# XiangFeng-Wen/STF-Unet

Measured on AMD Instinct MI355X. Metric: training samples/sec (256x256 DCE-MRI frames), higher is better.
Workload: dtype bf16; 1 GPU; cfg2 UNet(in=8,base_c=64) 256x256 train step; model=UNet, global_batch=64, per_gpu_batch=64, seq_len=8, parallelism=dp1, ddp_hook=False

## Files before the change

### include/stfunet.h

```cpp
#ifndef STFUNET_H
#define STFUNET_H
#include <stddef.h>
#include <stdint.h>

#ifdef __cplusplus
extern "C" {
#endif

typedef void* stf_stream_t;

typedef struct stf_conv_geom {
  int N;
  int Hs, Ws, Cs;
  int src_cstride;
  int Hd, Wd;
  int R, S;
  int stride, pad;
  int transposed;
} stf_conv_geom;

typedef struct stf_lstm_epi {
  const float* c_prev;
  float* c_out;
  void* h_out;
// ... 347 lines not shown
  int cx, cy, kx, ky;
  int oh, ow, h0, w0;
  int flags;
  int fx[6];
  int pad_;
  double m[6];
} stf_aug_frame;
int stf_augment_frames(const uint8_t* src, const stf_aug_frame* frames, int n, const int* coef,
                       uint8_t* scratch, int max_resized_px, int max_out_px, float mean, float stdv,
                       float* out, stf_stream_t stream);
int stf_augment_masks(const uint8_t* src, const stf_aug_frame* masks, int n, const int* tabs,
                      int max_out_px, int64_t* out, stf_stream_t stream);

typedef struct stf_plan stf_plan;
stf_plan* stf_plan_create(void);
void stf_plan_destroy(stf_plan* plan);
int stf_plan_record(stf_plan* plan);
int stf_plan_stop(void);
int stf_plan_size(const stf_plan* plan);
int stf_plan_tag(const char* name, double flops);
int stf_plan_tag_end(void);
int stf_plan_replay(stf_plan* plan, int first, int last, const char* timed_tag);
int stf_plan_timing(stf_plan* plan, int* launches, double* ms, double* flops);
int stf_stream_wait(stf_stream_t waiter, stf_stream_t waitee);
int stf_memset(void* p, int value, size_t bytes, stf_stream_t stream);
int stf_copy_rows(const float* src, int64_t src_ld, float* dst, int64_t dst_ld, int rows, int cols,
                  stf_stream_t stream);
int stf_i64_add_batch(int64_t* const* ptrs, int count, int64_t inc, stf_stream_t stream);

const char* stf_error_string(int code);
int stf_abi_version(void);

#define STF_STORAGE_BF16 0
#define STF_STORAGE_FP16 1
int stf_storage_type(void);

#ifdef __cplusplus
}
#endif
#endif
```

### stf-unet_amd/csrc/common.h

```cpp
#pragma once
#include <hip/hip_runtime.h>
#include <stdint.h>

#include <tuple>
#include <type_traits>
#include <utility>

#ifdef STF_FP16
typedef _Float16 e16;
#else
typedef __bf16 e16;
#endif
typedef e16 e16x8 __attribute__((ext_vector_type(8)));
typedef e16 e16x4 __attribute__((ext_vector_type(4)));
typedef short short4v __attribute__((ext_vector_type(4)));
typedef float f32x4 __attribute__((ext_vector_type(4)));
typedef float f32x16 __attribute__((ext_vector_type(16)));
typedef unsigned int u32x4v __attribute__((ext_vector_type(4)));

#define STF_DEV __device__ __forceinline__

STF_DEV float e2f(e16 v) { return (float)v; }
STF_DEV e16 f2e(float v) { return (e16)v; }

// ... 103 lines not shown
  return v;
}

template <typename T>
STF_DEV T wave_max(T v) {
#pragma unroll
  for (int o = 32; o > 0; o >>= 1) {
    const T t = __shfl_xor(v, o, 64);
    v = t > v ? t : v;
  }
  return v;
}
template <typename T>
STF_DEV T wave_min(T v) {
#pragma unroll
  for (int o = 32; o > 0; o >>= 1) {
    const T t = __shfl_xor(v, o, 64);
    v = t < v ? t : v;
  }
  return v;
}

namespace stf {
struct PlanOp {
  virtual ~PlanOp() {}
  virtual hipError_t run() const = 0;
};
bool plan_recording();
void plan_append(PlanOp* op, hipStream_t s);

template <class... A>
struct KernelOp final : PlanOp {
  const void* fn;
  dim3 grid, block;
  unsigned shmem;
  hipStream_t stream;
  std::tuple<A...> args;
  template <class... B>
  KernelOp(const void* f, dim3 g, dim3 b, unsigned sh, hipStream_t s, B&&... a)
      : fn(f), grid(g), block(b), shmem(sh), stream(s), args(std::forward<B>(a)...) {}
  hipError_t run() const override {
    return std::apply(
        [this](const A&... a) {
          void* p[sizeof...(A) + 1] = {const_cast<void*>(static_cast<const void*>(&a))...};
          return hipLaunchKernel(fn, grid, block, p, shmem, stream);
        },
        args);
  }
};

template <class... A, class... B>
inline void launch(void (*k)(A...), dim3 g, dim3 b, unsigned sh, hipStream_t s, B&&... args) {
  static_assert(sizeof...(A) == sizeof...(B), "kernel argument count");
  if (!plan_recording()) {
    std::tuple<std::decay_t<A>...> t(std::forward<B>(args)...);
    std::apply(
        [&](auto&... a) {
          void* p[sizeof...(A) + 1] = {static_cast<void*>(&a)...};
          (void)hipLaunchKernel((const void*)k, g, b, p, sh, s);
        },
        t);
    return;
  }
  auto* op = new KernelOp<std::decay_t<A>...>((const void*)k, g, b, sh, s, std::forward<B>(args)...);
  (void)op->run();
  plan_append(op, s);
}

hipError_t memset_async(void* p, int value, size_t bytes, hipStream_t s);
char ab_letter(const char* name);
hipError_t memcpy_async(void* dst, const void* src, size_t bytes, hipMemcpyKind kind, hipStream_t s);
// ... 25 lines not shown
```

### stf-unet_amd/csrc/head.hip

```cpp
#include "common.h"
#include "../../include/stfunet.h"
#include "reduce.h"

namespace {

constexpr int NT = 256;

STF_DEV float lane_group_sum(float v, int CG) {
  if (CG >= 2) v += dpp_f<0xB1>(v);
  if (CG >= 4) v += dpp_f<0x4E>(v);
  if (CG >= 8) v += dpp_f<0x141>(v);
  if (CG >= 16) v += dpp_f<0x140>(v);
  for (int o = 16; o < CG; o <<= 1) v += __shfl_xor(v, o, 64);
  return v;
}

int head_tiles(long units) {
  long t = (units + NT - 1) / NT;
  return (int)(t < 1 ? 1 : (t > 1024 ? 1024 : t));
}

template <int K>
__global__ void head_fwd_kernel(const uint16_t* __restrict__ y, long P, int HW, int C,
                                const float* __restrict__ scale, const float* __restrict__ shift,
// ... 345 lines not shown

extern "C" int stf_head_fwd(const void* y, int N, int H, int W, int C, const float* scale, const float* shift,
                            const float* w, const float* bias, int classes, float* logits, stf_stream_t stream) {
  if (!head_ok(C)) return STF_EINVAL;
  const long P = (long)N * H * W, units = P * (C / 8);
  if (units >= (1L << 31)) return STF_EINVAL;
  long blocks = (units + NT - 1) / NT;
  if (blocks > 8192) blocks = 8192;
  hipStream_t s = (hipStream_t)stream;
  STF_KDISPATCH(classes, hipLaunchKernelGGL(head_fwd_kernel<KK>, dim3(blocks), dim3(NT), 0, s, (const uint16_t*)y,
                                            P, H * W, C, scale, shift, w, bias, logits));
  STF_CHECK_LAUNCH();
  return 0;
}

extern "C" int stf_head_bwd(const float* dlogits, const void* y, int N, int H, int W, int C, const float* scale,
                            const float* shift, const float* mean, const float* invstd, const float* w, int classes,
                            void* g_out, float* bn_partial, float* head_partial, float* dw, float* db,
                            stf_stream_t stream) {
  if (!head_ok(C) || (long)N * H * W * (C / 8) >= (1L << 31)) return STF_EINVAL;
  const long P = (long)N * H * W;
  const int tiles = stf_head_tiles(N, H, W, C);
  hipStream_t s = (hipStream_t)stream;
  STF_KDISPATCH(classes, hipLaunchKernelGGL(head_bwd_kernel<KK>, dim3(tiles), dim3(NT), 0, s, dlogits,
                                            (const uint16_t*)y, P, H * W, C, scale, shift, mean, invstd, w,
                                            (uint16_t*)g_out, bn_partial, head_partial));
  STF_CHECK_LAUNCH();
  const int HC = classes * (C + 1);
  const int S = stf::colsum_stage1(head_partial, tiles, HC, s);
  hipLaunchKernelGGL(sum_tiles_kernel, dim3((HC + 255) / 256), dim3(256), 0, s, head_partial, S, HC, classes * C,
                     dw, db);
  STF_CHECK_LAUNCH();
  return 0;
}

extern "C" int stf_head_mc_fwd(const void* y, int N, int H, int W, int C, const float* scale, const float* shift,
                               const float* w, const float* bias, int classes, float* logits, stf_stream_t stream) {
  if (C < 8 || !head_ok(C) || !mc_classes_ok(classes) || N < 1 || H < 1 || W < 1) return STF_EINVAL;
  if (!y || !scale || !shift || !w || !bias || !logits) return STF_EINVAL;
  const long P = (long)N * H * W, units = P * (C / 8);
  if (!head_mc_units_ok((long)H * W, units)) return STF_EINVAL;
  long blocks = (units + NT - 1) / NT;
  if (blocks > MCBLOCKS) blocks = MCBLOCKS;
  hipStream_t s = (hipStream_t)stream;
  STF_KPDISPATCH(classes, hipLaunchKernelGGL(head_mc_fwd_kernel<KP>, dim3(blocks), dim3(NT),
                                             head_mc_lds_bytes(C, classes, false), s, (const uint16_t*)y, P, H * W, C,
// ... 30 lines not shown
```

### stf-unet_amd/csrc/loss.hip

```cpp
#include "common.h"
#include "../../include/stfunet.h"
#include <cmath>

namespace {

constexpr int NT = 256;
constexpr int MAXK = 4;
constexpr int MCK = 16;
constexpr int LCHUNK = 64;
constexpr float DICE_EPS = 1e-6f;

template <bool OPT> struct LossOpt { static constexpr int dice = 1; };
template <> struct LossOpt<true> { const float* cw; int ignore, dice; };

template <int K, bool OPT, class... O>
__global__ void loss_fwd_kernel(const float* __restrict__ logits, const int64_t* __restrict__ target, int HW,
                                float* __restrict__ part, O... opt) {
  constexpr int NV = 3 * K + 1 + OPT;
  const LossOpt<OPT> o{opt...};
  __shared__ float red[NT / 64][NV];
  const int n = blockIdx.y;
  float w[K];
  if constexpr (OPT) {
#pragma unroll
// ... 25 lines not shown
      s[3 * k] += p * tk;
      s[3 * k + 1] += p;
      s[3 * k + 2] += tk;
      if (t == k) {
        const float nll = lse - (z[k] - mx);
        if constexpr (OPT) { s[3 * K] += w[k] * nll; s[3 * K + 1] += w[k]; }
        else s[3 * K] += nll;
      }
    }
  }
#pragma unroll
  for (int i = 0; i < NV; ++i) s[i] = wave_sum(s[i]);
  if ((threadIdx.x & 63) == 0)
#pragma unroll
    for (int i = 0; i < NV; ++i) red[threadIdx.x >> 6][i] = s[i];
  __syncthreads();
  if (threadIdx.x < NV) {
    float a = 0.f;
    for (int wv = 0; wv < NT / 64; ++wv) a += red[wv][threadIdx.x];
    part[((size_t)n * gridDim.x + blockIdx.x) * NV + threadIdx.x] = a;
  }
}

template <int K, bool OPT>
__global__ void loss_finalize_kernel(const float* __restrict__ part, int N, int hw_or_dice, float* __restrict__ terms,
                                     float* __restrict__ loss) {
  constexpr int NV = 3 * K + 1 + OPT;
  __shared__ double acc[64][NV];
  double ce = 0.0, wsum = 0.0, dsum = 0.0;
  for (int base = 0; base < N; base += 64) {
    const int n = base + (int)threadIdx.x;
    if (threadIdx.x < 64) {
      for (int i = 0; i < NV; ++i) {
        double a = 0.0;
        if (n < N)
          for (int c = 0; c < LCHUNK; ++c) a += part[((size_t)n * LCHUNK + c) * NV + i];
        acc[threadIdx.x][i] = a;
      }
    }
    __syncthreads();
    if (threadIdx.x == 0) {
      for (int r = 0; r < 64 && base + r < N; ++r) {
        for (int k = 0; k < K; ++k) {
          const double I = acc[r][3 * k], S = acc[r][3 * k + 1] + acc[r][3 * k + 2];
          const float If = (float)I, Sf = (float)S;
          const float setsum = Sf == 0.f ? 2.f * If : Sf;
          dsum += (double)((2.f * If + DICE_EPS) / (setsum + DICE_EPS));
          terms[((size_t)(base + r) * K + k) * 3 + 0] = If;
          terms[((size_t)(base + r) * K + k) * 3 + 1] = (float)acc[r][3 * k + 1];
          terms[((size_t)(base + r) * K + k) * 3 + 2] = (float)acc[r][3 * k + 2];
        }
        ce += acc[r][3 * K];
        if constexpr (OPT) wsum += acc[r][3 * K + 1];
      }
    }
    __syncthreads();
  }
  if (threadIdx.x == 0) {
    terms[(size_t)N * K * 3] = (float)ce;
    if constexpr (OPT) {
      terms[(size_t)N * K * 3 + 1] = (float)wsum;
      loss[0] = (float)(ce / wsum + (hw_or_dice ? 1.0 - dsum / ((double)N * K) : 0.0));
    } else {
      loss[0] = (float)(ce / ((double)N * hw_or_dice) + 1.0 - dsum / ((double)N * K));
    }
  }
}

template <int K, bool OPT, class... O>
__global__ void loss_bwd_kernel(const float* __restrict__ logits, const int64_t* __restrict__ target, int N, int HW,
                                const float* __restrict__ terms, const float* __restrict__ grad_out,
                                float* __restrict__ dlogits, O... opt) {
  const LossOpt<OPT> o{opt...};
  const long P = (long)N * HW;
  const float go = grad_out ? grad_out[0] : 1.f;
  float inv_den = 1.f / (float)P;
// ... 109 lines not shown
    }
  }
  s[3 * KP] = wave_sum(s[3 * KP]);
  s[3 * KP + 1] = wave_sum(s[3 * KP + 1]);
#pragma unroll
  for (int i = 0; i < 3 * KP; ++i)
    if (i < 3 * K) s[i] = wave_sum(s[i]);
  if ((threadIdx.x & 63) == 0) {
#pragma unroll
    for (int i = 0; i < 3 * KP; ++i)
      if (i < 3 * K) red[threadIdx.x >> 6][i] = s[i];
    red[threadIdx.x >> 6][3 * K] = s[3 * KP];
    red[threadIdx.x >> 6][3 * K + 1] = s[3 * KP + 1];
  }
  __syncthreads();
  if ((int)threadIdx.x < NV) {
    float a = 0.f;
    for (int wv = 0; wv < NT / 64; ++wv) a += red[wv][threadIdx.x];
    part[((size_t)n * gridDim.x + blockIdx.x) * NV + threadIdx.x] = a;
  }
}

template <bool FT, class... F>
__global__ __launch_bounds__(NT) void loss_mc_finalize_kernel(const float* __restrict__ part, int N, int K, int dice,
                                                              F... ft, float* __restrict__ terms,
                                                              float* __restrict__ loss) {
  constexpr int NVM = 3 * MCK + 2;
  __shared__ double acc[64][NVM];
  __shared__ double dk[64][MCK], drow[64];
  const int NV = 3 * K + 2, r = threadIdx.x & 63, q = threadIdx.x >> 6;
  double ce = 0.0, wsum = 0.0, dsum = 0.0;
  for (int base = 0; base < N; base += 64) {
    const int n = base + r, rows = N - base < 64 ? N - base : 64;
    for (int i = q; i < NV; i += NT / 64) {
      double a = 0.0;
      if (n < N)
        for (int c = 0; c < LCHUNK; ++c) a += part[((size_t)n * LCHUNK + c) * NV + i];
      acc[r][i] = a;
    }
    __syncthreads();
    for (int e = threadIdx.x; e < rows * K; e += NT) {
      const int rr = e / K, k = e - rr * K;
      if constexpr (FT) {
        const LossFT o{0.f, ft...};
        const float I = (float)acc[rr][3 * k], P = (float)acc[rr][3 * k + 1], T = (float)acc[rr][3 * k + 2];
        const float den = 2.f * (1.f - o.alpha - o.beta) * I + 2.f * o.alpha * P + 2.f * o.beta * T + DICE_EPS;
        dk[rr][k] = (P + T == 0.f) ? 1.0 : (double)((2.f * I + DICE_EPS) / den);
        float* tp = terms + ((size_t)(base + rr) * K + k) * 3;
        tp[0] = I;
        tp[1] = P;
        tp[2] = T;
      } else {
        const double I = acc[rr][3 * k], S = acc[rr][3 * k + 1] + acc[rr][3 * k + 2];
        const float If = (float)I, Sf = (float)S;
        const float setsum = Sf == 0.f ? 2.f * If : Sf;
        dk[rr][k] = (double)((2.f * If + DICE_EPS) / (setsum + DICE_EPS));
        float* tp = terms + ((size_t)(base + rr) * K + k) * 3;
        tp[0] = If;
        tp[1] = (float)acc[rr][3 * k + 1];
        tp[2] = (float)acc[rr][3 * k + 2];
      }
    }
    __syncthreads();
    if ((int)threadIdx.x < rows) {
// ... 102 lines not shown
    }
#pragma unroll
    for (int k = 0; k < KP; ++k) {
      if (k < K) {
        const float tk = t == k ? 1.f : 0.f;
        const float G = (t == k ? ga[k] : 0.f) + gb[k];
        const float g = go * ((z[k] - tk) * cs + z[k] * (G - pg));
        dp[(size_t)k * HW + hw] = keep ? g : 0.f;
      }
    }
  }
}

int loss_scratch_floats(int N, int K, bool opt) { return N * K * 3 + 1 + opt + N * LCHUNK * (3 * K + 1 + opt); }

template <bool OPT, class... O>
int loss_fwd(const float* logits, const int64_t* target, int N, int HW, int classes, float* terms, float* loss,
             hipStream_t s, O... opt) {
  float* part = terms + N * classes * 3 + 1 + OPT;
  const int hw_or_dice = OPT ? LossOpt<OPT>{opt...}.dice : HW;
  STF_KDISPATCH(classes, {
    hipLaunchKernelGGL((loss_fwd_kernel<KK, OPT, O...>), dim3(LCHUNK, N), dim3(NT), 0, s, logits, target, HW, part,
                       opt...);
    hipLaunchKernelGGL((loss_finalize_kernel<KK, OPT>), dim3(1), dim3(64), 0, s, part, N, hw_or_dice, terms, loss);
  });
  STF_CHECK_LAUNCH();
  return 0;
}

template <bool OPT, class... O>
int loss_bwd(const float* logits, const int64_t* target, int N, int HW, int classes, const float* terms,
             const float* grad_out, float* dlogits, hipStream_t s, O... opt) {
  const long P = (long)N * HW;
  long blocks = (P + NT - 1) / NT;
  if (blocks > 8192) blocks = 8192;
  STF_KDISPATCH(classes, hipLaunchKernelGGL((loss_bwd_kernel<KK, OPT, O...>), dim3(blocks), dim3(NT), 0, s, logits,
                                            target, N, HW, terms, grad_out, dlogits, opt...));
  STF_CHECK_LAUNCH();
  return 0;
}

bool loss_opt_ok(int classes, int ignore_index) {
  return classes >= 1 && classes <= MAXK && !(ignore_index >= 0 && ignore_index < classes);
}

bool mc_classes_ok(int classes) { return classes >= 1 && classes <= MCK; }

bool loss_mc_ok(int N, int H, int W, int classes, int ignore_index) {
  return mc_classes_ok(classes) && !(ignore_index >= 0 && ignore_index < classes) && N >= 1 && N <= 65535 && H >= 1 &&
         W >= 1 && (long)H * W < (1L << 31);
}
bool loss_ft_ok() { return true; }
bool loss_ft_ok(float gamma, float alpha, float beta) {
  return std::isfinite(gamma) && gamma >= 0.f && std::isfinite(alpha) && alpha >= 0.f && std::isfinite(beta) &&
         beta >= 0.f && !(alpha == 0.f && beta == 0.f);
}

template <bool FT, class... F>
int loss_mc_fwd(const float* logits, const int64_t* target, int N, int H, int W, int classes, const float* cw,
                int ignore, int dice, float* terms, float* loss, hipStream_t s, F... ft) {
  if (!loss_mc_ok(N, H, W, classes, ignore) || !loss_ft_ok(ft...) || !logits || !target || !terms || !loss)
    return STF_EINVAL;
  float* part = terms + (size_t)N * classes * 3 + 2;
  const dim3 grid(LCHUNK, N);
  if constexpr (FT) {
    const LossFT o{ft...};
    STF_KPDISPATCH(classes, hipLaunchKernelGGL((loss_mc_fwd_kernel<KP, true, float>), grid, dim3(NT), 0, s, logits,
                                               target, H * W, classes, cw, ignore, o.gamma, part));
    hipLaunchKernelGGL((loss_mc_finalize_kernel<true, float, float>), dim3(1), dim3(NT), 0, s, part, N, classes,
                       dice, o.alpha, o.beta, terms, loss);
  } else {
    STF_KPDISPATCH(classes, hipLaunchKernelGGL((loss_mc_fwd_kernel<KP, false>), grid, dim3(NT), 0, s, logits, target,
                                               H * W, classes, cw, ignore, part));
    hipLaunchKernelGGL((loss_mc_finalize_kernel<false>), dim3(1), dim3(NT), 0, s, part, N, classes, dice, terms,
                       loss);
  }
  STF_CHECK_LAUNCH();
  return 0;
}

template <bool FT, class... F>
int loss_mc_bwd(const float* logits, const int64_t* target, int N, int H, int W, int classes, const float* cw,
                int ignore, int dice, const float* terms, const float* grad_out, float* dlogits, hipStream_t s,
                F... ft) {
  if (!loss_mc_ok(N, H, W, classes, ignore) || !loss_ft_ok(ft...) || !logits || !target || !terms || !dlogits)
    return STF_EINVAL;
  const int HW = H * W;
  long blocks = (HW + NT - 1) / NT, cap = 8192 / N;
  if (cap < 1) cap = 1;
  if (blocks > cap) blocks = cap;
  STF_KPDISPATCH(classes, hipLaunchKernelGGL((loss_mc_bwd_kernel<KP, FT, F...>), dim3(blocks, N), dim3(NT), 0, s,
                                             logits, target, N, HW, classes, cw, ignore, dice, ft..., terms,
                                             grad_out, dlogits));
  STF_CHECK_LAUNCH();
  return 0;
}

// ... 65 lines not shown
```

### stf-unet_amd/csrc/misc.hip

```cpp
#include "common.h"
#include "../../include/stfunet.h"
#include "reduce.h"

__global__ void stf_tile_sum_kernel(const float* __restrict__ partial, int tiles, int C, float* __restrict__ out);

namespace {

constexpr int NT = 256;

__global__ void adamw_kernel(float* __restrict__ p, const float* __restrict__ g, float* __restrict__ m,
                             float* __restrict__ v, long n, float lr, float b1, float b2, float eps, float wd,
                             float step_size, float inv_sqrt_bc2) {
  const long n4 = n / 4;
  for (long i = blockIdx.x * (long)NT + threadIdx.x; i < n4; i += (long)gridDim.x * NT) {
    float4 pv = reinterpret_cast<float4*>(p)[i];
    const float4 gv = reinterpret_cast<const float4*>(g)[i];
    float4 mv = reinterpret_cast<float4*>(m)[i];
    float4 vv = reinterpret_cast<float4*>(v)[i];
    float* pp = &pv.x; const float* gg = &gv.x; float* mm = &mv.x; float* ww = &vv.x;
#pragma unroll
    for (int j = 0; j < 4; ++j) {
      pp[j] *= 1.f - lr * wd;
      mm[j] = mm[j] + (1.f - b1) * (gg[j] - mm[j]);
      ww[j] = b2 * ww[j] + (1.f - b2) * gg[j] * gg[j];
// ... 8 lines not shown
    const float gg = g[i];
    const float mm = m[i] + (1.f - b1) * (gg - m[i]);
    const float ww = b2 * v[i] + (1.f - b2) * gg * gg;
    pp -= step_size * mm / (sqrtf(ww) * inv_sqrt_bc2 + eps);
    p[i] = pp; m[i] = mm; v[i] = ww;
  }
}

__global__ void pack_input_kernel(const float* __restrict__ x, int N, int C, int H, int W, int Cpad,
                                  uint16_t* __restrict__ out) {
  const int HW = H * W, P = N * HW;
  const int CG = Cpad / 8;
  for (int u = blockIdx.x * NT + threadIdx.x; u < P * CG; u += gridDim.x * NT) {
    const int cg = u / P;
    const int pix = u - cg * P;
    const int n = pix / HW, hw = pix - n * HW;
    float v[8];
#pragma unroll
    for (int j = 0; j < 8; ++j) {
      const int c = cg * 8 + j;
      v[j] = c < C ? x[((size_t)n * C + c) * HW + hw] : 0.f;
    }
    *reinterpret_cast<uint4*>(out + (size_t)pix * Cpad + cg * 8) = pack8(v);
  }
}

STF_DEV float pack_src(const float* __restrict__ w, int d0, int d1, int R, int S, int mode, int cpad, int o) {
  const int RS = R * S;
  if (mode == 0) {
    const int t = o / cpad, c = o - t * cpad;
    const int co = t / RS, tap = t - co * RS;
    return c < d1 ? w[(co * d1 + c) * RS + tap] : 0.f;
  } else if (mode == 1) {
    const int t = o / d0, co = o - t * d0;
    const int ci = t / RS, tap = t - ci * RS;
    return w[(co * d1 + ci) * RS + tap];
  } else if (mode == 2) {
    const int t = o / d0, ci = o - t * d0;
    const int tap = t / d1, co = t - tap * d1;
    return w[(ci * d1 + co) * RS + tap];
  } else if (mode == 3) {
    const int t = o / d1, co = o - t * d1;
    const int ci = t / RS, tap = t - ci * RS;
    return w[(ci * d1 + co) * RS + tap];
  } else if (mode == 5) {
    const int t = o / d0, co = o - t * d0;
// ... 238 lines not shown
  hipLaunchKernelGGL(adamw_clip_step_kernel, dim3(1), dim3(64), 0, (hipStream_t)stream, hyper, found_inf, clip);
  STF_CHECK_LAUNCH();
  if (n == 0) return 0;
  hipLaunchKernelGGL(adamw_clip_kernel, dim3(grid_for(n, 4096)), dim3(NT), 0, (hipStream_t)stream, p, g, m, v, (long)n,
                     hyper, beta1, beta2, eps, weight_decay, grad_scale, found_inf, clip);
  STF_CHECK_LAUNCH();
  return 0;
}

extern "C" int stf_adamw(float* p, const float* g, float* m, float* v, int64_t n, float lr, float beta1, float beta2,
                         float eps, float weight_decay, float bc1, float bc2, stf_stream_t stream) {
  if (((uintptr_t)p | (uintptr_t)g | (uintptr_t)m | (uintptr_t)v) & 15) return STF_EINVAL;
  const long blocks = grid_for(n / 4 + 1, 4096);
  hipLaunchKernelGGL(adamw_kernel, dim3(blocks), dim3(NT), 0, (hipStream_t)stream, p, g, m, v, (long)n, lr, beta1,
                     beta2, eps, weight_decay, lr / bc1, 1.f / sqrtf(bc2));
  STF_CHECK_LAUNCH();
  return 0;
}

extern "C" int stf_pack_input(const float* x, int N, int C, int H, int W, int Cpad, void* out, stf_stream_t stream) {
  if (Cpad % 8 || Cpad < C) return STF_EINVAL;
  const long units = (long)N * H * W * (Cpad / 8);
  if (units >= (1L << 31)) return STF_EINVAL;
  hipLaunchKernelGGL(pack_input_kernel, dim3(grid_for(units, 8192)), dim3(NT), 0, (hipStream_t)stream, x, N, C, H,
                     W, Cpad, (uint16_t*)out);
  STF_CHECK_LAUNCH();
  return 0;
}

extern "C" int stf_pack_weight(const float* w, int d0, int d1, int R, int S, int mode, int cpad, void* out,
                               stf_stream_t stream) {
  if (mode < 0 || mode > 5 || (mode == 0 && cpad < d1)) return STF_EINVAL;
  const long total = mode == 0 ? (long)d0 * R * S * cpad : (long)d0 * d1 * R * S;
  if (total >= (1L << 31) || (long)d0 * d1 * R * S >= (1L << 31)) return STF_EINVAL;
  hipLaunchKernelGGL(pack_weight_kernel, dim3(grid_for(total, 4096)), dim3(NT), 0, (hipStream_t)stream, w, d0, d1,
                     R, S, mode, cpad, (uint16_t*)out);
  STF_CHECK_LAUNCH();
  return 0;
}

extern "C" int stf_pack_tiles(int d0, int d1, int R, int S, int mode, int cpad) {
  const int RS = R * S;
  if (RS > PK_MAXRS || mode < 0 || mode > 5) return -1;
  const bool outer = mode == 1 || mode == 5 || mode == 2 || mode == 4;
  const int bext = mode == 0 ? cpad : d1;
  if (outer ? (d0 % 8) : (bext % 8)) return -1;
// ... 68 lines not shown
```

### stf-unet_amd/csrc/plan.hip

```cpp
#include "common.h"
#include "../../include/stfunet.h"

#include <atomic>
#include <cstdio>
#include <cstdlib>
#include <map>
#include <memory>
#include <mutex>
#include <string>
#include <vector>

namespace {

struct TagRange {
  int first, last;
  std::string name;
  double flops;
};

}

struct stf_plan {
  std::vector<std::unique_ptr<stf::PlanOp>> ops;
  std::vector<hipStream_t> op_stream;
  std::vector<TagRange> tags;
  int open_tag = -1;
  std::vector<std::pair<hipEvent_t, hipEvent_t>> ev;
  std::vector<int> ev_range;
  size_t ev_used = 0;
  ~stf_plan() {
    for (auto& e : ev) {
      (void)hipEventDestroy(e.first);
      (void)hipEventDestroy(e.second);
    }
  }
};

namespace {

thread_local stf_plan* g_rec = nullptr;

struct MemsetOp final : stf::PlanOp {
  void* p;
  int value;
  size_t bytes;
  hipStream_t s;
  hipError_t run() const override { return hipMemsetAsync(p, value, bytes, s); }
};

struct MemcpyOp final : stf::PlanOp {
  void* dst;
  const void* src;
  size_t bytes;
  hipStream_t s;
  hipError_t run() const override { return hipMemcpyAsync(dst, src, bytes, hipMemcpyDeviceToDevice, s); }
};

struct WaitOp final : stf::PlanOp {
  hipEvent_t ev = nullptr;
  hipStream_t waiter, waitee;
  ~WaitOp() override {
    if (ev) (void)hipEventDestroy(ev);
  }
  hipError_t run() const override {
    hipError_t e = hipEventRecord(ev, waitee);
    return e != hipSuccess ? e : hipStreamWaitEvent(waiter, ev, 0);
  }
};

void append(stf::PlanOp* op, hipStream_t s) {
  g_rec->ops.emplace_back(op);
  g_rec->op_stream.push_back(s);
}

std::mutex g_pool_mu;
std::map<int, std::vector<hipEvent_t>> g_pool;
std::map<int, unsigned> g_pool_next;
constexpr int POOL = 64;

hipError_t pooled_event(hipEvent_t* out) {
  int dev = 0;
  hipError_t e = hipGetDevice(&dev);
  if (e != hipSuccess) return e;
  std::lock_guard<std::mutex> g(g_pool_mu);
  auto& v = g_pool[dev];
  if (v.size() < POOL) {
    hipEvent_t ev;
    e = hipEventCreateWithFlags(&ev, hipEventDisableTiming);
    if (e != hipSuccess) return e;
    v.push_back(ev);
    *out = ev;
    return hipSuccess;
  }
// ... 20 lines not shown
__global__ void i64_add_kernel(I64Batch b, int n, int64_t inc) {
  if ((int)threadIdx.x < n) b.p[threadIdx.x][0] += inc;
}

}

bool stf::plan_recording() { return g_rec != nullptr; }

void stf::plan_append(stf::PlanOp* op, hipStream_t s) { append(op, s); }

char stf::ab_letter(const char* name) {
  const char* e = getenv(name);
  return e ? e[0] : 0;
}

hipError_t stf::memset_async(void* p, int value, size_t bytes, hipStream_t s) {
  if (!g_rec) return hipMemsetAsync(p, value, bytes, s);
  auto* op = new MemsetOp;
  op->p = p;
  op->value = value;
  op->bytes = bytes;
  op->s = s;
  hipError_t e = op->run();
  append(op, s);
  return e;
}

hipError_t stf::memcpy_async(void* dst, const void* src, size_t bytes, hipMemcpyKind kind, hipStream_t s) {
  if (!g_rec) return hipMemcpyAsync(dst, src, bytes, kind, s);
  if (kind != hipMemcpyDeviceToDevice) return hipErrorInvalidValue;
  auto* op = new MemcpyOp;
  op->dst = dst;
  op->src = src;
  op->bytes = bytes;
  op->s = s;
  hipError_t e = op->run();
  append(op, s);
  return e;
}

extern "C" stf_plan* stf_plan_create(void) { return new stf_plan; }

extern "C" void stf_plan_destroy(stf_plan* p) { delete p; }

extern "C" int stf_plan_record(stf_plan* p) {
  if (!p || g_rec) return STF_EINVAL;
  p->ops.clear();
  p->op_stream.clear();
  p->tags.clear();
  p->open_tag = -1;
  g_rec = p;
  return 0;
}

extern "C" int stf_plan_stop(void) {
  if (!g_rec) return STF_EINVAL;
  if (g_rec->open_tag >= 0) g_rec->tags[g_rec->open_tag].last = (int)g_rec->ops.size();
  g_rec->open_tag = -1;
  g_rec = nullptr;
  return 0;
}

extern "C" int stf_plan_size(const stf_plan* p) { return p ? (int)p->ops.size() : -1; }

extern "C" int stf_plan_tag(const char* name, double flops) {
  if (!g_rec || !name) return 0;
  stf_plan* p = g_rec;
  if (p->open_tag >= 0) p->tags[p->open_tag].last = (int)p->ops.size();
  p->tags.push_back(TagRange{(int)p->ops.size(), -1, name, flops});
  p->open_tag = (int)p->tags.size() - 1;
  return 0;
}

extern "C" int stf_plan_tag_end(void) {
  if (!g_rec || g_rec->open_tag < 0) return 0;
// ... 127 lines not shown
```

### stf-unet_amd/stfunet/_lib.py

```python
import contextlib
import ctypes
import os

import torch

_HERE = os.path.dirname(os.path.abspath(__file__))
LIB_PATH = os.path.join(_HERE, "libstfunet_hip.so")
LIB_PATH = os.environ.get("STF_LIB", LIB_PATH)
LIB_PATH_F16 = os.environ.get("STF_LIB_F16", os.path.join(os.path.dirname(LIB_PATH), "libstfunet_hip_f16.so"))
LIB_PATHS = {torch.bfloat16: LIB_PATH, torch.float16: LIB_PATH_F16}
STORAGE_CODE = {torch.bfloat16: 0, torch.float16: 1}

BUILD_INFO = os.path.join(_HERE, "build_info.json")
_SRC_DIRS = (os.path.join(_HERE, "..", "csrc"), os.path.join(_HERE, "..", "..", "include"))


def _sha(paths):
    import hashlib
    h = hashlib.sha256()
    for p in paths:
        h.update(os.path.basename(p).encode())
        with open(p, "rb") as f:
            h.update(f.read())
    return h.hexdigest()[:16]
# ... 186 lines not shown
    "stf_stem_dgrad7": (c_int, [P, P, c_int, c_int, c_int, c_int, c_int, c_int, P, P]),
    "stf_maxpool3s2_fwd": (c_int, [P, c_int, c_int, c_int, c_int, P, P, P]),
    "stf_maxpool3s2_bwd": (c_int, [P, P, c_int, c_int, c_int, c_int, P, P]),
    "stf_bn_act_maxpool3s2": (c_int, [P, c_int, c_int, c_int, c_int, c_int, P, P, P, P, P]),
    "stf_bn_bwd_reduce_pool3": (c_int, [P, P, P, c_int, c_int, c_int, c_int, c_int, P, P, P, P, P, P]),
    "stf_bn_bwd_apply_pool3": (c_int, [P, P, P, c_int, c_int, c_int, c_int, c_int, P, P, P, P, P]),
    "stf_lstm_pack": (c_int, [P, P, P, P, c_int, P, P, P, P]),
    "stf_lstm_unpack_grad": (c_int, [P, P, c_int, P, P, P, P, P]),
    "stf_lstm_seq_fwd": (c_int, [P, P, P, c_int, c_int, c_int, P, P, c_int, P]),
    "stf_lstm_seq_supported": (c_int, [c_int]),
    "stf_lstm_seq_bwd": (c_int, [P, P, P, P, c_int, c_int, c_int, P, P, c_int, P, P, c_int, P]),
    "stf_lstm_cell_bwd": (c_int, [P, P, P, P, c_int, P, P, P, c_int64, c_int, P]),
    "stf_pk_resize": (c_int, [P, c_int, c_int, c_int, c_int, c_int, c_int, c_int, c_int, P, c_int, c_int, P]),
    "stf_plan_create": (c_void_p, []),
    "stf_plan_destroy": (None, [P]),
    "stf_plan_record": (c_int, [P]),
    "stf_plan_stop": (c_int, []),
    "stf_plan_size": (c_int, [P]),
    "stf_plan_tag": (c_int, [ctypes.c_char_p, ctypes.c_double]),
    "stf_plan_tag_end": (c_int, []),
    "stf_plan_replay": (c_int, [P, c_int, c_int, ctypes.c_char_p]),
    "stf_plan_timing": (c_int, [P, ctypes.POINTER(c_int), ctypes.POINTER(ctypes.c_double),
                                ctypes.POINTER(ctypes.c_double)]),
    "stf_stream_wait": (c_int, [P, P]),
    "stf_memset": (c_int, [P, c_int, c_size_t, P]),
    "stf_copy_rows": (c_int, [P, c_int64, P, c_int64, c_int, c_int, P]),
    "stf_i64_add_batch": (c_int, [ctypes.POINTER(c_void_p), c_int, c_int64, P]),
    "stf_error_string": (ctypes.c_char_p, [c_int]),
    "stf_abi_version": (c_int, []),
    "stf_storage_type": (c_int, []),
}

EXPORTED = tuple(_SIGS)
_libs = {}
_active = torch.bfloat16
_FNS = {}
_FN = _FNS.setdefault(_active, {})


def load(dtype=None):
    dtype = _active if dtype is None else dtype
    lib = _libs.get(dtype)
    if lib is not None:
        return lib
    if dtype not in LIB_PATHS:
        raise ValueError(f"no stfunet library for storage dtype {dtype} (bf16 or fp16)")
    path = LIB_PATHS[dtype]
    if not os.path.exists(path):
        raise RuntimeError(f"stfunet HIP library not built ({path}); run `make -C stf-unet_amd/csrc` "
                           "or __graft_entry__.build()")
    lib = ctypes.CDLL(path)
    for name, (res, args) in _SIGS.items():
        fn = getattr(lib, name)
        fn.restype = res
        fn.argtypes = args
    if lib.stf_storage_type() != STORAGE_CODE[dtype]:
        raise RuntimeError(f"{path} was built for another storage type ({lib.stf_storage_type()})")
    _libs[dtype] = lib
    return lib


def storage_dtype():
    return _active


def storage_for(requested=None):
    if requested is not None:
        return requested
    if torch.is_autocast_enabled("cuda") and torch.get_autocast_dtype("cuda") == torch.float16:
        return torch.float16
    return torch.bfloat16


@contextlib.contextmanager
def storage(dtype):
    global _active, _FN
    if dtype not in LIB_PATHS:
        raise ValueError(f"activation storage must be torch.bfloat16 or torch.float16, not {dtype}")
    prev = _active
    _active, _FN = dtype, _FNS.setdefault(dtype, {})
    try:
        yield
# ... 41 lines not shown
```

### stf-unet_amd/stfunet/plan.py

```python
import contextlib
import ctypes
import gc
import os
import threading
import weakref
from collections import OrderedDict

import torch

from . import _lib, nhwc
from ._lib import call

TIMED = None
RECORD_HOOK = None

_POOL_LOCK = threading.RLock()
_POOL_ACTIVE = 0
_GRAVEYARD = []


POOL_EVENTS = {"buried": 0, "destroyed": 0, "entry_del": 0}


def _bury(pool):
    if pool is not None:
        with _POOL_LOCK:
            _GRAVEYARD.append(pool)
            POOL_EVENTS["buried"] += 1


def drain_pools():
    with _POOL_LOCK:
        if _POOL_ACTIVE or not _GRAVEYARD:
            return
        dead = _GRAVEYARD[:]
        _GRAVEYARD.clear()
        POOL_EVENTS["destroyed"] += len(dead)
        dead.clear()


@contextlib.contextmanager
def _pool_context(pool):
    global _POOL_ACTIVE
    if pool is None:
# ... 9 lines not shown
            _POOL_ACTIVE -= 1
        drain_pools()


def _stf_env():
    data = getattr(os.environ, "_data", None)
    if isinstance(data, dict):
        return tuple(sorted((k, v) for k, v in data.items() if k.startswith(b"STF_")))
    return tuple(sorted((k, v) for k, v in os.environ.items() if k.startswith("STF_")))


def enabled():
    return os.environ.get("STF_PLAN", "1") != "0" and not torch.cuda.is_current_stream_capturing()


class Plan:

    def __init__(self):
        self.lib = _lib.load()
        self.h = self.lib.stf_plan_create()
        if not self.h:
            raise MemoryError("stf_plan_create failed")
        self.n = 0

    def record(self, fn):
        _lib.check(self.lib.stf_plan_record(self.h), "stf_plan_record")
        nhwc.RECORDING = True
        try:
            return fn()
        finally:
            nhwc.RECORDING = False
            _lib.check(self.lib.stf_plan_stop(), "stf_plan_stop")
            self.n = self.lib.stf_plan_size(self.h)

    def size(self):
        return self.lib.stf_plan_size(self.h)

    def replay(self, first=0, last=None):
        last = self.n if last is None else last
        if last > first:
            tag = TIMED.encode() if TIMED is not None else None
            _lib.check(self.lib.stf_plan_replay(self.h, first, last, tag), "stf_plan_replay")

    def timing(self):
        n, ms, fl = ctypes.c_int(0), ctypes.c_double(0.0), ctypes.c_double(0.0)
        _lib.check(self.lib.stf_plan_timing(self.h, ctypes.byref(n), ctypes.byref(ms), ctypes.byref(fl)),
                   "stf_plan_timing")
        return n.value, ms.value, fl.value

    def __del__(self):
        h, self.h = getattr(self, "h", None), None
        if h:
            self.lib.stf_plan_destroy(h)


@contextlib.contextmanager
def _no_gc():
    was = gc.isenabled()
    gc.disable()
    try:
        yield
    finally:
        if was:
            gc.enable()


def _new_pool():
    if os.environ.get("STF_PLAN_POOL", "1") == "0" or not hasattr(torch.cuda, "MemPool"):
        return None
    return torch.cuda.MemPool()


class _Entry:

    def __init__(self):
        self.seen = 0
        self.fwd = self.bwd = None
        self.x = self.logits = self.S = None
        self.bsig = None
        self.dl = None
        self.marks = []
        self.keep = []
        self.bkeep = []
        self.pool = None
        self.owner = None

    def release(self):
        pool, self.pool = self.pool, None
        self.fwd = self.bwd = None
        self.x = self.logits = self.S = self.dl = None
        self.keep, self.bkeep = [], []
        _bury(pool)

    def __del__(self):
        POOL_EVENTS["entry_del"] += 1
        pool = getattr(self, "pool", None)
        if pool is not None:
            self.pool = None
            _bury(pool)

    def busy(self):
        o = self.owner() if self.owner is not None else None
        return o is not None and self.S is not None and getattr(o, "saved", None) is self.S


class StepRuntime:

    def __init__(self, prog):
        self._prog = weakref.ref(prog)
        self._bns = None
        self.warm = int(os.environ.get("STF_PLAN_WARM", "1"))
        self.slots = max(1, int(os.environ.get("STF_PLAN_SLOTS", "2")))
        self._bufs = None
# ... 45 lines not shown
                _, old = self.entries.popitem(last=False)
                if old is self.cur:
                    self.cur = None
                old.release()
            e = self.entries[sig] = _Entry()
        else:
            self.entries.move_to_end(sig)
        return e

    def forward(self, x, training, need_bwd, ctx=None):
        p = self.prog
        drain_pools()
        if not (enabled() and training and need_bwd and nhwc.TIMER is None):
            return p.forward(x, training, need_bwd)
        e = self._entry(self._signature(x, training))
        if e.busy():
            return p.forward(x, training, need_bwd)
        if e.fwd is None:
            e.seen += 1
            if e.seen <= self.warm:
                return p.forward(x, training, need_bwd)
            self._record_forward(e, x, training)
        else:
            e.x.copy_(x)
            e.fwd.replay()
        if ctx is not None:
            e.owner = weakref.ref(ctx)
        self.cur = e
        return e.logits, e.S

    def own(self, S, ctx):
        e = self.cur
        if e is not None and S is not None and e.S is S:
            e.owner = weakref.ref(ctx)

    def _record_forward(self, e, x, training):
        with _no_gc():
            self._record_forward_pooled(e, x, training)

    def _record_forward_pooled(self, e, x, training):
        e.pool = _new_pool()
        nhwc.KEEP = e.keep
        prog = self.prog

        def run():
            if RECORD_HOOK is not None:
                RECORD_HOOK(self, "forward")
            return prog.forward(e.x, training, True)
        try:
            with _pool_context(e.pool):
                e.x = nhwc.empty(tuple(x.shape), x.dtype, x.device)
                e.x.copy_(x)
                plan = Plan()
                e.logits, e.S = plan.record(run)
        finally:
            nhwc.KEEP = None
        e.fwd = plan

    def backward(self, S, dlogits):
        p = self.prog
        e = next((v for v in self.entries.values() if v.fwd is not None and v.S is S), None)
        if e is None or not enabled() or nhwc.TIMER is not None:
            return p.backward(S, dlogits)
        fmap = getattr(S, "fmap", None)
        bsig = (tuple(dlogits.shape), p.flat.grad.data_ptr(), p.grad_ready_hook is not None, _lib.stream(),
                fmap.key if fmap is not None else None)
        if e.bwd is None or bsig != e.bsig:
            return self._record_backward(e, S, dlogits, bsig)
        e.dl.copy_(dlogits)
        pos = 0
        hook = p.grad_ready_hook
        for idx, off, deps in e.marks:
            e.bwd.replay(pos, idx)
            hook(off, deps)
            pos = idx
        e.bwd.replay(pos)

    def _record_backward(self, e, S, dlogits, bsig):
        with _no_gc():
            self._record_backward_pooled(e, S, dlogits, bsig)

    def _record_backward_pooled(self, e, S, dlogits, bsig):
        p = self.prog
        e.bwd = None
        e.bkeep = []
        nhwc.KEEP = e.bkeep
        plan = Plan()
        marks = []
        real_hook = p.grad_ready_hook
        pend = []
        if real_hook is not None:
            def hook(off, deps=()):
                pend.extend(d for d in deps if all(d is not q for q in pend))
                acted = real_hook(off, deps)
                if acted is None or acted:
                    marks.append((plan.size(), off, tuple(pend)))
                    pend.clear()
            p.grad_ready_hook = hook

        def run():
            if RECORD_HOOK is not None:
                RECORD_HOOK(self, "backward")
            return p.backward(S, e.dl)
        try:
            with _pool_context(e.pool):
                e.dl = nhwc.empty(tuple(dlogits.shape), dlogits.dtype, dlogits.device)
                e.dl.copy_(dlogits)
                plan.record(run)
        finally:
            nhwc.KEEP = None
            p.grad_ready_hook = real_hook
        e.bwd, e.bsig, e.marks = plan, bsig, marks

    def timing(self):
        tot = [0, 0.0, 0.0]
        for e in self.entries.values():
            for pl in (e.fwd, e.bwd):
                if pl is not None:
                    n, ms, fl = pl.timing()
                    tot[0] += n
                    tot[1] += ms
                    tot[2] += fl
        return tuple(tot)
```

Before: 2715 samples/s.

## Bind plan inputs to live tensors, vectorize input packing and widen loss finalize

Adds pointer-slot binding to recorded launch plans so replay patches kernel arguments to read the caller's input and dlogits tensors directly, instead of copying them into static buffers first. It also adds a vectorized pack kernel for 8-channel inputs with width divisible by 4, using float4 loads and an LDS transpose. The single-block loss finalize kernels now run with 1024 threads and parallel chunk folding in place of a 64-thread serial loop. Argument scanning adds recording complexity, and any pointer use that cannot be patched falls back to the copy path.

Measured after the change: 2726 samples/s (median of 6 runs). About the same (+0.4%).

```diff
diff --git a/include/stfunet.h b/include/stfunet.h
--- a/include/stfunet.h
+++ b/include/stfunet.h
@@ -393,6 +393,10 @@
 int stf_plan_tag_end(void);
 int stf_plan_replay(stf_plan* plan, int first, int last, const char* timed_tag);
 int stf_plan_timing(stf_plan* plan, int* launches, double* ms, double* flops);
+int stf_plan_bind(int slot, const void* ptr, size_t bytes);
+int stf_plan_bound_refs(const stf_plan* plan, int slot);
+int stf_plan_replay_bound(stf_plan* plan, int first, int last, const char* timed_tag, const void* const* addrs,
+                          int count);
 int stf_stream_wait(stf_stream_t waiter, stf_stream_t waitee);
 int stf_memset(void* p, int value, size_t bytes, stf_stream_t stream);
 int stf_copy_rows(const float* src, int64_t src_ld, float* dst, int64_t dst_ld, int rows, int cols,
diff --git a/stf-unet_amd/csrc/common.h b/stf-unet_amd/csrc/common.h
--- a/stf-unet_amd/csrc/common.h
+++ b/stf-unet_amd/csrc/common.h
@@ -149,12 +149,24 @@
 }
 
 namespace stf {
+struct PlanArg {
+  void* at;
+  size_t bytes;
+  bool pointer, to_const;
+};
 struct PlanOp {
   virtual ~PlanOp() {}
   virtual hipError_t run() const = 0;
+  virtual int plan_args(PlanArg*, int) { return 0; }
 };
 bool plan_recording();
 void plan_append(PlanOp* op, hipStream_t s);
+struct PlanInputReader {
+  PlanInputReader();
+  ~PlanInputReader();
+  PlanInputReader(const PlanInputReader&) = delete;
+  PlanInputReader& operator=(const PlanInputReader&) = delete;
+};
 
 template <class... A>
 struct KernelOp final : PlanOp {
@@ -174,6 +186,18 @@
         },
         args);
   }
+  int plan_args(PlanArg* out, int cap) override {
+    int n = 0;
+    std::apply(
+        [&](A&... a) {
+          ((n < cap ? (void)(out[n++] = PlanArg{static_cast<void*>(&a), sizeof(A), std::is_pointer<A>::value,
+                                                std::is_const<std::remove_pointer_t<A>>::value})
+                    : (void)0),
+           ...);
+        },
+        this->args);
+    return n;
+  }
 };
 
 template <class... A, class... B>
diff --git a/stf-unet_amd/csrc/head.hip b/stf-unet_amd/csrc/head.hip
--- a/stf-unet_amd/csrc/head.hip
+++ b/stf-unet_amd/csrc/head.hip
@@ -391,6 +391,7 @@
   const long P = (long)N * H * W;
   const int tiles = stf_head_tiles(N, H, W, C);
   hipStream_t s = (hipStream_t)stream;
+  const stf::PlanInputReader reads_dlogits;
   STF_KDISPATCH(classes, hipLaunchKernelGGL(head_bwd_kernel<KK>, dim3(tiles), dim3(NT), 0, s, dlogits,
                                             (const uint16_t*)y, P, H * W, C, scale, shift, mean, invstd, w,
                                             (uint16_t*)g_out, bn_partial, head_partial));
diff --git a/stf-unet_amd/csrc/loss.hip b/stf-unet_amd/csrc/loss.hip
--- a/stf-unet_amd/csrc/loss.hip
+++ b/stf-unet_amd/csrc/loss.hip
@@ -71,36 +71,47 @@
   }
 }
 
+constexpr int FIN_NT = 1024;
+
+STF_DEV double fold_chunks(const float* __restrict__ p, int NV) {
+  float v[LCHUNK];
+#pragma unroll
+  for (int c = 0; c < LCHUNK; ++c) v[c] = p[(size_t)c * NV];
+  double a = 0.0;
+#pragma unroll
+  for (int c = 0; c < LCHUNK; ++c) a += v[c];
+  return a;
+}
+
 template <int K, bool OPT>
-__global__ void loss_finalize_kernel(const float* __restrict__ part, int N, int hw_or_dice, float* __restrict__ terms,
-                                     float* __restrict__ loss) {
+__global__ __launch_bounds__(FIN_NT) void loss_finalize_kernel(const float* __restrict__ part, int N, int hw_or_dice,
+                                                               float* __restrict__ terms, float* __restrict__ loss) {
   constexpr int NV = 3 * K + 1 + OPT;
+  static_assert(NV <= 16 && FIN_NT == 64 * 16, "thread (r, i): image base + r, value i of 16");
   __shared__ double acc[64][NV];
+  __shared__ double dk[64][K];
+  const int r = threadIdx.x >> 4, i = threadIdx.x & 15;
   double ce = 0.0, wsum = 0.0, dsum = 0.0;
   for (int base = 0; base < N; base += 64) {
-    const int n = base + (int)threadIdx.x;
-    if (threadIdx.x < 64) {
-      for (int i = 0; i < NV; ++i) {
-        double a = 0.0;
-        if (n < N)
-          for (int c = 0; c < LCHUNK; ++c) a += part[((size_t)n * LCHUNK + c) * NV + i];
-        acc[threadIdx.x][i] = a;
-      }
+    const int n = base + r;
+    if (i < NV) acc[r][i] = n < N ? fold_chunks(part + (size_t)n * LCHUNK * NV + i, NV) : 0.0;
+    __syncthreads();
+    if (i < K && n < N) {
+      const int k = i;
+      const double I = acc[r][3 * k], S = acc[r][3 * k + 1] + acc[r][3 * k + 2];
+      const float If = (float)I, Sf = (float)S;
+      const float setsum = Sf == 0.f ? 2.f * If : Sf;
+      dk[r][k] = (double)((2.f * If + DICE_EPS) / (setsum + DICE_EPS));
+      terms[((size_t)n * K + k) * 3 + 0] = If;
+      terms[((size_t)n * K + k) * 3 + 1] = (float)acc[r][3 * k + 1];
+      terms[((size_t)n * K + k) * 3 + 2] = (float)acc[r][3 * k + 2];
     }
     __syncthreads();
     if (threadIdx.x == 0) {
-      for (int r = 0; r < 64 && base + r < N; ++r) {
-        for (int k = 0; k < K; ++k) {
-          const double I = acc[r][3 * k], S = acc[r][3 * k + 1] + acc[r][3 * k + 2];
-          const float If = (float)I, Sf = (float)S;
-          const float setsum = Sf == 0.f ? 2.f * If : Sf;
-          dsum += (double)((2.f * If + DICE_EPS) / (setsum + DICE_EPS));
-          terms[((size_t)(base + r) * K + k) * 3 + 0] = If;
-          terms[((size_t)(base + r) * K + k) * 3 + 1] = (float)acc[r][3 * k + 1];
-          terms[((size_t)(base + r) * K + k) * 3 + 2] = (float)acc[r][3 * k + 2];
-        }
-        ce += acc[r][3 * K];
-        if constexpr (OPT) wsum += acc[r][3 * K + 1];
+      for (int rr = 0; rr < 64 && base + rr < N; ++rr) {
+        for (int k = 0; k < K; ++k) dsum += dk[rr][k];
+        ce += acc[rr][3 * K];
+        if constexpr (OPT) wsum += acc[rr][3 * K + 1];
       }
     }
     __syncthreads();
@@ -256,7 +267,7 @@
 }
 
 template <bool FT, class... F>
-__global__ __launch_bounds__(NT) void loss_mc_finalize_kernel(const float* __restrict__ part, int N, int K, int dice,
+__global__ __launch_bounds__(FIN_NT) void loss_mc_finalize_kernel(const float* __restrict__ part, int N, int K, int dice,
                                                               F... ft, float* __restrict__ terms,
                                                               float* __restrict__ loss) {
   constexpr int NVM = 3 * MCK + 2;
@@ -266,14 +277,10 @@
   double ce = 0.0, wsum = 0.0, dsum = 0.0;
   for (int base = 0; base < N; base += 64) {
     const int n = base + r, rows = N - base < 64 ? N - base : 64;
-    for (int i = q; i < NV; i += NT / 64) {
-      double a = 0.0;
-      if (n < N)
-        for (int c = 0; c < LCHUNK; ++c) a += part[((size_t)n * LCHUNK + c) * NV + i];
-      acc[r][i] = a;
-    }
-    __syncthreads();
-    for (int e = threadIdx.x; e < rows * K; e += NT) {
+    for (int i = q; i < NV; i += FIN_NT / 64)
+      acc[r][i] = n < N ? fold_chunks(part + (size_t)n * LCHUNK * NV + i, NV) : 0.0;
+    __syncthreads();
+    for (int e = threadIdx.x; e < rows * K; e += FIN_NT) {
       const int rr = e / K, k = e - rr * K;
       if constexpr (FT) {
         const LossFT o{0.f, ft...};
@@ -422,7 +429,7 @@
   STF_KDISPATCH(classes, {
     hipLaunchKernelGGL((loss_fwd_kernel<KK, OPT, O...>), dim3(LCHUNK, N), dim3(NT), 0, s, logits, target, HW, part,
                        opt...);
-    hipLaunchKernelGGL((loss_finalize_kernel<KK, OPT>), dim3(1), dim3(64), 0, s, part, N, hw_or_dice, terms, loss);
+    hipLaunchKernelGGL((loss_finalize_kernel<KK, OPT>), dim3(1), dim3(FIN_NT), 0, s, part, N, hw_or_dice, terms, loss);
   });
   STF_CHECK_LAUNCH();
   return 0;
@@ -467,12 +474,12 @@
     const LossFT o{ft...};
     STF_KPDISPATCH(classes, hipLaunchKernelGGL((loss_mc_fwd_kernel<KP, true, float>), grid, dim3(NT), 0, s, logits,
                                                target, H * W, classes, cw, ignore, o.gamma, part));
-    hipLaunchKernelGGL((loss_mc_finalize_kernel<true, float, float>), dim3(1), dim3(NT), 0, s, part, N, classes,
+    hipLaunchKernelGGL((loss_mc_finalize_kernel<true, float, float>), dim3(1), dim3(FIN_NT), 0, s, part, N, classes,
                        dice, o.alpha, o.beta, terms, loss);
   } else {
     STF_KPDISPATCH(classes, hipLaunchKernelGGL((loss_mc_fwd_kernel<KP, false>), grid, dim3(NT), 0, s, logits, target,
                                                H * W, classes, cw, ignore, part));
-    hipLaunchKernelGGL((loss_mc_finalize_kernel<false>), dim3(1), dim3(NT), 0, s, part, N, classes, dice, terms,
+    hipLaunchKernelGGL((loss_mc_finalize_kernel<false>), dim3(1), dim3(FIN_NT), 0, s, part, N, classes, dice, terms,
                        loss);
   }
   STF_CHECK_LAUNCH();
diff --git a/stf-unet_amd/csrc/misc.hip b/stf-unet_amd/csrc/misc.hip
--- a/stf-unet_amd/csrc/misc.hip
+++ b/stf-unet_amd/csrc/misc.hip
@@ -54,6 +54,46 @@
       v[j] = c < C ? x[((size_t)n * C + c) * HW + hw] : 0.f;
     }
     *reinterpret_cast<uint4*>(out + (size_t)pix * Cpad + cg * 8) = pack8(v);
+  }
+}
+
+constexpr int PI_PIX = 4 * NT;
+__global__ __launch_bounds__(NT) void pack_input_w4_kernel(const float* __restrict__ x, int P, int C, int HW,
+                                                           uint16_t* __restrict__ out) {
+  __shared__ uint4 tile[PI_PIX];
+  const int p0 = blockIdx.x * PI_PIX, tid = threadIdx.x;
+  if ((reinterpret_cast<uintptr_t>(x) & 15) == 0) {
+    const int p = p0 + 4 * tid;
+    if (p < P) {
+      const int n = p / HW, hw = p - n * HW;
+      const float* src = x + (size_t)n * C * HW + hw;
+      float4 q[8];
+#pragma unroll
+      for (int j = 0; j < 8; ++j)
+        q[j] = j < C ? *reinterpret_cast<const float4*>(src + (size_t)j * HW) : make_float4(0.f, 0.f, 0.f, 0.f);
+      float v[4][8];
+#pragma unroll
+      for (int j = 0; j < 8; ++j) { v[0][j] = q[j].x; v[1][j] = q[j].y; v[2][j] = q[j].z; v[3][j] = q[j].w; }
+#pragma unroll
+      for (int i = 0; i < 4; ++i) tile[4 * tid + i] = pack8(v[i]);
+    }
+    __syncthreads();
+#pragma unroll
+    for (int i = 0; i < 4; ++i) {
+      const int pix = p0 + i * NT + tid;
+      if (pix < P) *reinterpret_cast<uint4*>(out + (size_t)pix * 8) = tile[i * NT + tid];
+    }
+  } else {
+#pragma unroll
+    for (int i = 0; i < 4; ++i) {
+      const int pix = p0 + i * NT + tid;
+      if (pix >= P) continue;
+      const int n = pix / HW, hw = pix - n * HW;
+      float v[8];
+#pragma unroll
+      for (int j = 0; j < 8; ++j) v[j] = j < C ? x[((size_t)n * C + j) * HW + hw] : 0.f;
+      *reinterpret_cast<uint4*>(out + (size_t)pix * 8) = pack8(v);
+    }
   }
 }
 
@@ -338,6 +378,14 @@
   if (Cpad % 8 || Cpad < C) return STF_EINVAL;
   const long units = (long)N * H * W * (Cpad / 8);
   if (units >= (1L << 31)) return STF_EINVAL;
+  const stf::PlanInputReader reads_x;
+  if (Cpad == 8 && W % 4 == 0) {
+    const int P = (int)units;
+    hipLaunchKernelGGL(pack_input_w4_kernel, dim3((P + PI_PIX - 1) / PI_PIX), dim3(NT), 0, (hipStream_t)stream, x, P,
+                       C, H * W, (uint16_t*)out);
+    STF_CHECK_LAUNCH();
+    return 0;
+  }
   hipLaunchKernelGGL(pack_input_kernel, dim3(grid_for(units, 8192)), dim3(NT), 0, (hipStream_t)stream, x, N, C, H,
                      W, Cpad, (uint16_t*)out);
   STF_CHECK_LAUNCH();
diff --git a/stf-unet_amd/csrc/plan.hip b/stf-unet_amd/csrc/plan.hip
--- a/stf-unet_amd/csrc/plan.hip
+++ b/stf-unet_amd/csrc/plan.hip
@@ -4,6 +4,7 @@
 #include <atomic>
 #include <cstdio>
 #include <cstdlib>
+#include <cstring>
 #include <map>
 #include <memory>
 #include <mutex>
@@ -18,6 +19,19 @@
   double flops;
 };
 
+constexpr int MAX_SLOTS = 4;
+struct BoundRef {
+  int op;
+  void** at;
+  size_t delta;
+};
+struct BoundSlot {
+  uintptr_t base = 0;
+  size_t bytes = 0;
+  bool bound = false, poisoned = false;
+  std::vector<BoundRef> refs;
+};
+
 }
 
 struct stf_plan {
@@ -25,6 +39,7 @@
   std::vector<hipStream_t> op_stream;
   std::vector<TagRange> tags;
   int open_tag = -1;
+  BoundSlot slots[MAX_SLOTS];
   std::vector<std::pair<hipEvent_t, hipEvent_t>> ev;
   std::vector<int> ev_range;
   size_t ev_used = 0;
@@ -39,6 +54,41 @@
 namespace {
 
 thread_local stf_plan* g_rec = nullptr;
+thread_local int g_input_reader = 0;
+
+void note_address(uintptr_t value, void** at, bool patchable) {
+  for (BoundSlot& b : g_rec->slots) {
+    if (!b.bound || value < b.base || value - b.base >= b.bytes) continue;
+    if (patchable) b.refs.push_back(BoundRef{(int)g_rec->ops.size(), at, (size_t)(value - b.base)});
+    else b.poisoned = true;
+  }
+}
+
+bool any_bound() {
+  for (const BoundSlot& b : g_rec->slots)
+    if (b.bound) return true;
+  return false;
+}
+
+void scan_args(stf::PlanOp* op) {
+  if (!any_bound()) return;
+  stf::PlanArg a[64];
+  const int n = op->plan_args(a, 64);
+  for (int i = 0; i < n; ++i) {
+    if (a[i].pointer) {
+      void** at = static_cast<void**>(a[i].at);
+      note_address(reinterpret_cast<uintptr_t>(*at), at, a[i].to_const && g_input_reader > 0);
+    } else {
+      for (size_t o = 0; o + sizeof(uintptr_t) <= a[i].bytes; o += sizeof(uintptr_t)) {
+        uintptr_t v;
+        memcpy(&v, static_cast<const char*>(a[i].at) + o, sizeof v);
+        note_address(v, nullptr, false);
+      }
+    }
+  }
+  if (n == 64)
+    for (BoundSlot& b : g_rec->slots) b.poisoned = b.poisoned || b.bound;
+}
 
 struct MemsetOp final : stf::PlanOp {
   void* p;
@@ -69,6 +119,7 @@
 };
 
 void append(stf::PlanOp* op, hipStream_t s) {
+  scan_args(op);
   g_rec->ops.emplace_back(op);
   g_rec->op_stream.push_back(s);
 }
@@ -135,6 +186,7 @@
   op->bytes = bytes;
   op->s = s;
   hipError_t e = op->run();
+  note_address(reinterpret_cast<uintptr_t>(p), nullptr, false);
   append(op, s);
   return e;
 }
@@ -148,9 +200,14 @@
   op->bytes = bytes;
   op->s = s;
   hipError_t e = op->run();
+  note_address(reinterpret_cast<uintptr_t>(dst), nullptr, false);
+  note_address(reinterpret_cast<uintptr_t>(src), nullptr, false);
   append(op, s);
   return e;
 }
+
+stf::PlanInputReader::PlanInputReader() { ++g_input_reader; }
+stf::PlanInputReader::~PlanInputReader() { --g_input_reader; }
 
 extern "C" stf_plan* stf_plan_create(void) { return new stf_plan; }
 
@@ -162,8 +219,41 @@
   p->op_stream.clear();
   p->tags.clear();
   p->open_tag = -1;
+  for (BoundSlot& b : p->slots) b = BoundSlot();
   g_rec = p;
   return 0;
+}
+
+extern "C" int stf_plan_bind(int slot, const void* ptr, size_t bytes) {
+  if (!g_rec || slot < 0 || slot >= MAX_SLOTS || !ptr || !bytes) return STF_EINVAL;
+  BoundSlot& b = g_rec->slots[slot];
+  if (b.bound || !g_rec->ops.empty()) return STF_EINVAL;
+  b.base = reinterpret_cast<uintptr_t>(ptr);
+  b.bytes = bytes;
+  b.bound = true;
+  return 0;
+}
+
+extern "C" int stf_plan_bound_refs(const stf_plan* p, int slot) {
+  if (!p || slot < 0 || slot >= MAX_SLOTS) return -1;
+  const BoundSlot& b = p->slots[slot];
+  return (!b.bound || b.poisoned) ? -1 : (int)b.refs.size();
+}
+
+extern "C" int stf_plan_replay_bound(stf_plan* p, int first, int last, const char* timed_tag,
+                                     const void* const* addrs, int count) {
+  if (!p || g_rec == p || !addrs || count < 0 || count > MAX_SLOTS) return STF_EINVAL;
+  for (int i = 0; i < count; ++i) {
+    const BoundSlot& b = p->slots[i];
+    if (!addrs[i]) continue;
+    if (!b.bound || b.poisoned) return STF_EINVAL;
+  }
+  for (int i = 0; i < count; ++i) {
+    if (!addrs[i]) continue;
+    for (const BoundRef& r : p->slots[i].refs)
+      *r.at = reinterpret_cast<void*>(reinterpret_cast<uintptr_t>(addrs[i]) + r.delta);
+  }
+  return stf_plan_replay(p, first, last, timed_tag);
 }
 
 extern "C" int stf_plan_stop(void) {
diff --git a/stf-unet_amd/stfunet/_lib.py b/stf-unet_amd/stfunet/_lib.py
--- a/stf-unet_amd/stfunet/_lib.py
+++ b/stf-unet_amd/stfunet/_lib.py
@@ -232,6 +232,9 @@
     "stf_plan_replay": (c_int, [P, c_int, c_int, ctypes.c_char_p]),
     "stf_plan_timing": (c_int, [P, ctypes.POINTER(c_int), ctypes.POINTER(ctypes.c_double),
                                 ctypes.POINTER(ctypes.c_double)]),
+    "stf_plan_bind": (c_int, [c_int, P, c_size_t]),
+    "stf_plan_bound_refs": (c_int, [P, c_int]),
+    "stf_plan_replay_bound": (c_int, [P, c_int, c_int, ctypes.c_char_p, ctypes.POINTER(c_void_p), c_int]),
     "stf_stream_wait": (c_int, [P, P]),
     "stf_memset": (c_int, [P, c_int, c_size_t, P]),
     "stf_copy_rows": (c_int, [P, c_int64, P, c_int64, c_int, c_int, P]),
@@ -242,6 +245,7 @@
 }
 
 EXPORTED = tuple(_SIGS)
+_LATER = ("stf_plan_bind", "stf_plan_bound_refs", "stf_plan_replay_bound")
 _libs = {}
 _active = torch.bfloat16
 _FNS = {}
@@ -261,6 +265,8 @@
                            "or __graft_entry__.build()")
     lib = ctypes.CDLL(path)
     for name, (res, args) in _SIGS.items():
+        if name in _LATER and not hasattr(lib, name):
+            continue
         fn = getattr(lib, name)
         fn.restype = res
         fn.argtypes = args
@@ -268,6 +274,10 @@
         raise RuntimeError(f"{path} was built for another storage type ({lib.stf_storage_type()})")
     _libs[dtype] = lib
     return lib
+
+
+def has(name, dtype=None):
+    return hasattr(load(dtype), name)
 
 
 def storage_dtype():
diff --git a/stf-unet_amd/stfunet/plan.py b/stf-unet_amd/stfunet/plan.py
--- a/stf-unet_amd/stfunet/plan.py
+++ b/stf-unet_amd/stfunet/plan.py
@@ -20,6 +20,7 @@
 
 
 POOL_EVENTS = {"buried": 0, "destroyed": 0, "entry_del": 0}
+BIND_EVENTS = {"x_bound": 0, "x_copied": 0, "dl_bound": 0, "dl_copied": 0}
 
 
 def _bury(pool):
@@ -75,16 +76,22 @@
         if not self.h:
             raise MemoryError("stf_plan_create failed")
         self.n = 0
-
-    def record(self, fn):
+        self.bound = False
+
+    def record(self, fn, bind=None):
         _lib.check(self.lib.stf_plan_record(self.h), "stf_plan_record")
+        can_bind = bind is not None and _lib.has("stf_plan_bind")
         nhwc.RECORDING = True
         try:
+            if can_bind:
+                _lib.check(self.lib.stf_plan_bind(0, bind.data_ptr(), bind.numel() * bind.element_size()),
+                           "stf_plan_bind")
             return fn()
         finally:
             nhwc.RECORDING = False
             _lib.check(self.lib.stf_plan_stop(), "stf_plan_stop")
             self.n = self.lib.stf_plan_size(self.h)
+            self.bound = can_bind and self.lib.stf_plan_bound_refs(self.h, 0) > 0
 
     def size(self):
         return self.lib.stf_plan_size(self.h)
@@ -94,6 +101,12 @@
         if last > first:
             tag = TIMED.encode() if TIMED is not None else None
             _lib.check(self.lib.stf_plan_replay(self.h, first, last, tag), "stf_plan_replay")
+
+    def replay_at(self, addr, first=0, last=None):
+        last = self.n if last is None else last
+        tag = TIMED.encode() if TIMED is not None else None
+        slot = (ctypes.c_void_p * 1)(addr)
+        _lib.check(self.lib.stf_plan_replay_bound(self.h, first, last, tag, slot, 1), "stf_plan_replay_bound")
 
     def timing(self):
         n, ms, fl = ctypes.c_int(0), ctypes.c_double(0.0), ctypes.c_double(0.0)
@@ -137,11 +150,13 @@
         self.bkeep = []
         self.pool = None
         self.owner = None
+        self.x_live = self.dl_live = None
 
     def release(self):
         pool, self.pool = self.pool, None
         self.fwd = self.bwd = None
         self.x = self.logits = self.S = self.dl = None
+        self.x_live = self.dl_live = None
         self.keep, self.bkeep = [], []
         _bury(pool)
 
@@ -233,12 +248,27 @@
                 return p.forward(x, training, need_bwd)
             self._record_forward(e, x, training)
         else:
-            e.x.copy_(x)
-            e.fwd.replay()
+            e.x_live = self._feed(e.fwd, e.x, x, "x")
         if ctx is not None:
             e.owner = weakref.ref(ctx)
         self.cur = e
         return e.logits, e.S
+
+    @staticmethod
+    def _feed(plan, static, t, what, last=None):
+        if plan.bound:
+            if t.is_contiguous() and t.dtype == static.dtype and t.data_ptr() % 16 == 0 and t.numel() == static.numel():
+                BIND_EVENTS[what + "_bound"] += 1
+                plan.replay_at(t.data_ptr(), 0, last)
+                return t
+            static.copy_(t)
+            BIND_EVENTS[what + "_copied"] += 1
+            plan.replay_at(static.data_ptr(), 0, last)
+            return None
+        static.copy_(t)
+        BIND_EVENTS[what + "_copied"] += 1
+        plan.replay(0, last)
+        return None
 
     def own(self, S, ctx):
         e = self.cur
@@ -263,7 +293,7 @@
                 e.x = nhwc.empty(tuple(x.shape), x.dtype, x.device)
                 e.x.copy_(x)
                 plan = Plan()
-                e.logits, e.S = plan.record(run)
+                e.logits, e.S = plan.record(run, bind=e.x)
         finally:
             nhwc.KEEP = None
         e.fwd = plan
@@ -278,14 +308,16 @@
                 fmap.key if fmap is not None else None)
         if e.bwd is None or bsig != e.bsig:
             return self._record_backward(e, S, dlogits, bsig)
-        e.dl.copy_(dlogits)
-        pos = 0
         hook = p.grad_ready_hook
-        for idx, off, deps in e.marks:
-            e.bwd.replay(pos, idx)
+        pos = e.marks[0][0] if e.marks else None
+        e.dl_live = self._feed(e.bwd, e.dl, dlogits, "dl", pos)
+        for k, (idx, off, deps) in enumerate(e.marks):
+            if k:
+                e.bwd.replay(pos, idx)
             hook(off, deps)
             pos = idx
-        e.bwd.replay(pos)
+        if e.marks:
+            e.bwd.replay(pos)
 
     def _record_backward(self, e, S, dlogits, bsig):
         with _no_gc():
@@ -294,6 +326,7 @@
     def _record_backward_pooled(self, e, S, dlogits, bsig):
         p = self.prog
         e.bwd = None
+        e.dl_live = None
         e.bkeep = []
         nhwc.KEEP = e.bkeep
         plan = Plan()
@@ -317,7 +350,7 @@
             with _pool_context(e.pool):
                 e.dl = nhwc.empty(tuple(dlogits.shape), dlogits.dtype, dlogits.device)
                 e.dl.copy_(dlogits)
-                plan.record(run)
+                plan.record(run, bind=e.dl)
         finally:
             nhwc.KEEP = None
             p.grad_ready_hook = real_hook
```
